# mlelarge/graph_neural_net

Measured on AMD Instinct MI355X. Metric: graph-pairs/sec FGNN fwd+bwd, N=50 regular pairs, higher is better.
Workload: dtype f32

## Files before the change

graph_neural_net_amd/csrc/mlp_fwd.hip:

```cpp
#include "fgnn_common.h"
#include "fgnn_pack.h"

#ifdef FGNN_PHASES
__device__ unsigned long long *g_fwd_stamp = nullptr;
__device__ int g_fwd_sel = 0;
#endif

namespace {

constexpr int TLD = 36;
constexpr int TILE_F = 32 * TLD;

struct TileCtx {
    int g, tt, p, i, jj;
    bool inb;
};

DEVI TileCtx decode_tile(int tile, bool active, int tpg, int N, int P, int j) {
    TileCtx c;
    c.g = __builtin_amdgcn_readfirstlane(active ? tile / tpg : 0);
    c.tt = active ? tile - c.g * tpg : 0;
    c.p = c.tt * FGNN_TILE + j;
    c.inb = active && c.p < P;
    c.i = c.p / N;
    c.jj = c.p - c.i * N;
    return c;
}
DEVI bool tile_valid(const TileCtx &c, int nv) { return c.inb && c.i < nv && c.jj < nv; }

template <int S>
DEVI constexpr int slab_ch(int k, int h) { return S == 16 ? ch_of(k, h) : 2 * k + h; }
template <int S>
DEVI constexpr int slab_kbase(int k) { return S == 16 ? (k & 3) + 8 * (k >> 2) : 2 * k; }
template <int S>
DEVI constexpr int slab_hmul() { return S == 16 ? 4 : 1; }

template <int HMUL>
DEVI int lane_off(const View &v, const TileCtx &c, int h) {
    return c.inb ? HMUL * h * v.ld4 + 4 * c.p : OOB_OFF;
}

template <int S>
DEVI void load_raw(float (&x)[S > 0 ? S : 1], const View &v, const TileCtx &c, int h) {
    if constexpr (S > 0) {
        const int voff = lane_off<slab_hmul<S>()>(v, c, h);
        const int s0 = c.g * v.gs4;
#pragma unroll
        for (int k = 0; k < S; ++k) x[k] = buf_load(v, voff, s0 + slab_kbase<S>(k) * v.ld4);
    }
}

template <int S, bool PK>
DEVI void load_slab(float (&x)[S > 0 ? S : 1], const View &v, const PackedSrc &ps, const TileCtx &c, int h) {
    if constexpr (PK && S == 1) load_packed(x, ps, c, h);
    else load_raw<S>(x, v, c, h);
}

template <int S>
DEVI void apply_norm(float (&x)[S > 0 ? S : 1], const float *rec, bool on, bool valid, int h) {
    if constexpr (S > 0) {
        if (on) {
            const float4 *r4 = reinterpret_cast<const float4 *>(rec);
            const float vf = valid ? 1.f : 0.f;
#pragma unroll
            for (int k = 0; k < S; ++k) {
                const float4 n = r4[slab_ch<S>(k, h)];
                x[k] = ((x[k] - n.x) * n.y + n.z) * vf;
            }
        }
    }
}

template <int CA, int CB>
constexpr int fwd_waves() { return 16; }

template <int CA, int CB, int NMLP, int DEPTH>
struct FwdLayout {
    static constexpr int NW = fwd_waves<CA, CB>();
    static constexpr int SA = CA / 2, SB = CB / 2;
    static constexpr int pad4(int x) { return (x + 3) & ~3; }
    static constexpr PkFwd PK = pk_fwd(CA, CB, DEPTH);
    static constexpr int OFF_W1A = PK.off_w1a;
    static constexpr int OFF_W1B = PK.off_w1b;
    static constexpr int OFF_WH = PK.off_wh;
    static constexpr int BIAS_F = PK.bias_f;
    static constexpr int MLP_STEPS = PK.steps;
    static constexpr int MLP_F = PK.floats;
    static constexpr int WEIGHT_F = NMLP * MLP_F;
    static constexpr int REC_F = 2 * 32 * 4;
    static constexpr int LDS_F = WEIGHT_F + NW * (TILE_F + REC_F);
};

template <int CNT>
DEVI void load_ops(float (&dst)[CNT > 0 ? CNT : 1], const float *wl, int off_steps, int lane) {
    const float4 *p = reinterpret_cast<const float4 *>(wl) + (off_steps / 4) * 64 + lane;
#pragma unroll
    for (int q = 0; q < (CNT + 3) / 4; ++q) {
        const float4 v = p[q * 64];
        if (4 * q + 0 < CNT) dst[4 * q + 0] = v.x;
        if (4 * q + 1 < CNT) dst[4 * q + 1] = v.y;
        if (4 * q + 2 < CNT) dst[4 * q + 2] = v.z;
        if (4 * q + 3 < CNT) dst[4 * q + 3] = v.w;
    }
}

DEVI void load_bias(float (&dst)[16], const float *tail, int layer, int h) {
    const float4 *p = reinterpret_cast<const float4 *>(tail + layer * 32 + h * 16);
#pragma unroll
    for (int q = 0; q < 4; ++q) {
        const float4 v = p[q];
        dst[4 * q + 0] = v.x;
        dst[4 * q + 1] = v.y;
        dst[4 * q + 2] = v.z;
        dst[4 * q + 3] = v.w;
    }
}

template <int CA, int CB, int NMLP, int DEPTH, bool PK, bool SKIP, bool DBG>
DEVI void mlp_fwd_body(const fgnn_mlp_fwd_args A, const int tpg, const int total_tiles, unsigned *const dbg0, unsigned *const dbg1) {
    extern __shared__ __attribute__((aligned(16))) float smem[];
    using L = FwdLayout<CA, CB, NMLP, DEPTH>;
    constexpr int NW = L::NW;
#ifdef FGNN_PHASES
    const unsigned long long st0_ = __builtin_amdgcn_s_memtime();
    unsigned long long st1_ = 0;
    int ntl_ = 0;
#endif
    constexpr int SA = CA / 2, SB = CB / 2;
    const int lane = threadIdx.x & 63, wv = __builtin_amdgcn_readfirstlane(threadIdx.x >> 6);
    const int j = lane & 31, h = lane >> 5;
    const int P = A.N * A.N;
    float *wl = smem;
    float *tl = smem + L::WEIGHT_F + wv * TILE_F;
    float *recA = smem + L::WEIGHT_F + NW * TILE_F + wv * L::REC_F, *recB = recA + 128;
    const View va = make_view(A.a.ptr, A.a.gstride, A.a.ldp, A.G);
    const View vb = make_view(A.b.ptr, A.b.gstride, A.b.ldp, A.G);
    PackedSrc ps = {};
    if constexpr (PK) ps = make_packed_src(A.xbits, A.xdeg, A.G, A.N);
    View vz[NMLP];
#pragma unroll
    for (int m = 0; m < NMLP; ++m) vz[m] = make_view(A.z[m], FGNN_H * A.ldz, A.ldz, A.G);

    const int nwg = gridDim.x;
    const int q = total_tiles / nwg, rem = total_tiles % nwg;
    int T0 = blockIdx.x * q + ((int)blockIdx.x < rem ? (int)blockIdx.x : rem);
    int T1 = T0 + q + ((int)blockIdx.x < rem ? 1 : 0);
    if constexpr (SKIP) {
        T0 = A.ranges[blockIdx.x];
        T1 = A.ranges[blockIdx.x + 1];
    }

    const bool normA = A.a.nrm != nullptr, normB = (CB > 0) && A.b.nrm != nullptr;
    int *live_list = reinterpret_cast<int *>(smem + L::LDS_F);
    int nlive = 0, li = wv, live_cnt = 0;
    bool use_list = false;
    if constexpr (SKIP) {
        nlive = build_live_list(live_list, live_list + LIVE_LIST_CAP, T0, T1, tpg, FGNN_TILE, A.N, A.nvalid, threadIdx.x, 64 * NW);
        use_list = nlive <= LIVE_LIST_CAP;
    }
    auto next_tile = [&](int cur, bool first) {
        if constexpr (SKIP) {
            if (use_list) {
                if (!first) li += NW;
                return __builtin_amdgcn_readfirstlane(li < nlive ? live_list[li] : T1);
            }
            return __builtin_amdgcn_readfirstlane(next_owned_live_tile_p(first ? T0 : cur + 1, T1, live_cnt, wv, NW, tpg, FGNN_TILE, A.N, A.nvalid));
        } else {
            return first ? T0 + wv : cur + NW;
        }
    };
    PkRegs<L::WEIGHT_F / 4, 64 * NW> img;
    if (A.packed) pk_load_regs(img, A.packed);
    __builtin_amdgcn_sched_barrier(0);
    int tile = next_tile(0, true);
    float xa[SA > 0 ? SA : 1], xb[SB > 0 ? SB : 1];
    float4 ra = make_float4(0.f, 0.f, 0.f, 0.f), rb = ra;
    int cached_g = -1, cur_nv = A.N;
    {
        const TileCtx c = decode_tile(tile, tile < T1, tpg, A.N, P, j);
        load_slab<SA, PK>(xa, va, ps, c, h);
        load_slab<SB, PK>(xb, vb, ps, c, h);
        if (tile < T1 && lane < 32) {
            if (normA && lane < CA) {
                ra = reinterpret_cast<const float4 *>(A.a.nrm)[(long long)c.g * A.a.C + lane];
                ra.z = A.a.beta ? A.a.beta[lane] : 0.f;
            }
            if (normB && lane < CB) {
                rb = reinterpret_cast<const float4 *>(A.b.nrm)[(long long)c.g * A.b.C + lane];
                rb.z = A.b.beta ? A.b.beta[lane] : 0.f;
            }
        }
        if (tile < T1) {
            cached_g = c.g;
            cur_nv = __builtin_amdgcn_readfirstlane(nvalid_of(A.nvalid, c.g, A.N));
        }
    }
    if (A.packed) {
        pk_store_regs(wl, img);
    } else {
        constexpr PkFwd pk = L::PK;
#pragma unroll
        for (int m = 0; m < NMLP; ++m) {
            const float *Wp[FGNN_MAX_DEPTH] = {A.W[m][0], A.W[m][1], A.W[m][2]};
            const float *Bp[FGNN_MAX_DEPTH] = {A.bias[m][0], A.bias[m][1], A.bias[m][2]};
            for (int e = threadIdx.x; e < L::MLP_F; e += 64 * NW) {
                if (e < L::BIAS_F) {
                    const int t = e >> 6, l = e & 63;
                    wl[m * L::MLP_F + (t >> 2) * 256 + l * 4 + (t & 3)] = pk_fwd_value(pk, CA, CB, Wp, t, l);
                } else {
                    wl[m * L::MLP_F + e] = pk_bias_value(Bp, e - L::BIAS_F);
                }
            }
        }
    }
    if (lane < 32) {
        reinterpret_cast<float4 *>(recA)[lane] = ra;
        reinterpret_cast<float4 *>(recB)[lane] = rb;
    }
    __syncthreads();
#ifdef FGNN_PHASES
    st1_ = __builtin_amdgcn_s_memtime();
#endif

    while (tile < T1) {
#ifdef FGNN_PHASES
        ++ntl_;
#endif
        const TileCtx c = decode_tile(tile, true, tpg, A.N, P, j);
        if (c.g != cached_g) {
            if (lane < 32) {
                if (normA && lane < CA) {
                    float4 n = reinterpret_cast<const float4 *>(A.a.nrm)[(long long)c.g * A.a.C + lane];
                    n.z = A.a.beta ? A.a.beta[lane] : 0.f;
                    reinterpret_cast<float4 *>(recA)[lane] = n;
                }
                if (normB && lane < CB) {
                    float4 n = reinterpret_cast<const float4 *>(A.b.nrm)[(long long)c.g * A.b.C + lane];
                    n.z = A.b.beta ? A.b.beta[lane] : 0.f;
                    reinterpret_cast<float4 *>(recB)[lane] = n;
                }
            }
            cached_g = c.g;
            cur_nv = __builtin_amdgcn_readfirstlane(nvalid_of(A.nvalid, c.g, A.N));
        }
        const bool c_valid = tile_valid(c, cur_nv);
        const int next = next_tile(tile, false);
        float na[SA > 0 ? SA : 1], nb[SB > 0 ? SB : 1];
        {
            const TileCtx cn = decode_tile(next, next < T1, tpg, A.N, P, j);
            load_slab<SA, PK>(na, va, ps, cn, h);
            load_slab<SB, PK>(nb, vb, ps, cn, h);
        }
        apply_norm<SA>(xa, recA, normA, c_valid, h);
        apply_norm<SB>(xb, recB, normB, c_valid, h);

        const unsigned vmask = (unsigned)__ballot(c_valid);
        const float cnt = (float)__popc(vmask);
        const float inv = cnt > 0.f ? 1.f / cnt : 0.f;
#pragma unroll
        for (int m = 0; m < NMLP; ++m) {
            const float *wm = wl + m * L::MLP_F;
            f32x16 acc;
            {
                float b0[16];
                load_bias(b0, wm + L::BIAS_F, 0, h);
#pragma unroll
                for (int r = 0; r < 16; ++r) acc[r] = b0[r];
                float w1a[SA > 0 ? SA : 1];
                load_ops<SA>(w1a, wm, L::OFF_W1A, lane);
#pragma unroll
                for (int s = 0; s < SA; ++s) acc = mfma32(w1a[s], xa[s], acc);
                if constexpr (SB > 0) {
                    float w1b[SB > 0 ? SB : 1];
                    load_ops<SB>(w1b, wm, L::OFF_W1B, lane);
#pragma unroll
                    for (int s = 0; s < SB; ++s) acc = mfma32(w1b[s], xb[s], acc);
                }
            }
#pragma unroll
            for (int l = 1; l < DEPTH; ++l) {
                float hid[16], bl[16], wh[16];
                load_bias(bl, wm + L::BIAS_F, l, h);
                load_ops<16>(wh, wm, L::OFF_WH + 16 * (l - 1), lane);
                if constexpr (DBG) {
#pragma unroll
                    for (int r = 0; r < 16; ++r) {
                        const unsigned long long mk = __ballot(__float_as_int(acc[r]) > 0);
                        if (lane == 0) {
                            unsigned *o = (m == 0 ? dbg0 : dbg1) + (((long long)c.g * (DEPTH - 1) + (l - 1)) * 32 + ch_of(r, 0)) * tpg + c.tt;
                            o[0] = (unsigned)mk;
                            o[4ll * tpg] = (unsigned)(mk >> 32);
                        }
                    }
                }
#pragma unroll
                for (int r = 0; r < 16; ++r) {
                    hid[r] = relu1(acc[r]);
                    acc[r] = bl[r];
                }
#pragma unroll
                for (int r = 0; r < 16; ++r) acc = mfma32(wh[r], hid[r], acc);
            }
            const int zoff = lane_off<4>(vz[m], c, h);
            const int zs0 = c.g * vz[m].gs4;
#pragma unroll
            for (int r = 0; r < 16; ++r) {
                const int chl = (r & 3) + 8 * (r >> 2);
                const float v = c_valid ? acc[r] : 0.f;
                buf_store(v, vz[m], zoff, zs0 + chl * vz[m].ld4);
                tl[(chl + 4 * h) * TLD + j] = v;
            }
            const float4 *rp = reinterpret_cast<const float4 *>(tl + j * TLD + 16 * h);
            float4 qv[4];
#pragma unroll
            for (int k = 0; k < 4; ++k) qv[k] = rp[k];
            float s = 0.f;
#pragma unroll
            for (int k = 0; k < 4; ++k) s += (qv[k].x + qv[k].y) + (qv[k].z + qv[k].w);
            s += __shfl_xor(s, 32);
            const float mean = s * inv;
            const unsigned mh = vmask >> (16 * h);
            float m2 = 0.f;
#pragma unroll
            for (int k = 0; k < 4; ++k) {
                const float d0 = ((mh >> (4 * k + 0)) & 1u) ? qv[k].x - mean : 0.f;
                const float d1 = ((mh >> (4 * k + 1)) & 1u) ? qv[k].y - mean : 0.f;
                const float d2 = ((mh >> (4 * k + 2)) & 1u) ? qv[k].z - mean : 0.f;
                const float d3 = ((mh >> (4 * k + 3)) & 1u) ? qv[k].w - mean : 0.f;
                m2 += (d0 * d0 + d1 * d1) + (d2 * d2 + d3 * d3);
            }
            m2 += __shfl_xor(m2, 32);
            if (h == 0) {
                float2 o;
                o.x = mean;
                o.y = m2;
                reinterpret_cast<float2 *>(A.part[m])[((long long)c.g * tpg + c.tt) * FGNN_H + j] = o;
            }
        }
        if (lane == 0) A.cnt[(long long)c.g * tpg + c.tt] = cnt;

#pragma unroll
        for (int s = 0; s < SA; ++s) xa[s] = na[s];
#pragma unroll
        for (int s = 0; s < SB; ++s) xb[s] = nb[s];
        tile = next;
    }
    if constexpr (SKIP) {
        for (int t = T0 + wv; t < T1; t += NW) {
            const TileCtx c = decode_tile(t, true, tpg, A.N, P, j);
            if (tile_live(c.tt, A.N, A.nvalid[c.g])) continue;
#pragma unroll
            for (int m = 0; m < NMLP; ++m) {
                if (h == 0)
                    reinterpret_cast<float2 *>(A.part[m])[((long long)c.g * tpg + c.tt) * FGNN_H + j] = make_float2(0.f, 0.f);
            }
            if (lane == 0) A.cnt[(long long)c.g * tpg + c.tt] = 0.f;
        }
    }
#ifdef FGNN_PHASES
    if (g_fwd_stamp && g_fwd_sel == CA * 1000 + CB * 10 + NMLP && (threadIdx.x & 63) == 0) {
        unsigned long long *o = g_fwd_stamp + ((long long)blockIdx.x * NW + wv) * 4;
        o[0] = st0_;
        o[1] = st1_;
        o[2] = __builtin_amdgcn_s_memtime();
        o[3] = ntl_;
    }
#endif
}

template <int CA, int CB, int NMLP, int DEPTH, bool PK = false, bool SKIP = false>
__global__ __launch_bounds__((64 * fwd_waves<CA, CB>()), (fwd_waves<CA, CB>() / 4)) void mlp_fwd_kernel(
    const fgnn_mlp_fwd_args A, const int tpg, const int total_tiles) {
    mlp_fwd_body<CA, CB, NMLP, DEPTH, PK, SKIP, false>(A, tpg, total_tiles, nullptr, nullptr);
}
template <int CA, int CB, int NMLP, int DEPTH, bool PK = false, bool SKIP = false>
__global__ __launch_bounds__((64 * fwd_waves<CA, CB>()), (fwd_waves<CA, CB>() / 4)) void mlp_fwd_dbg_kernel(
    const fgnn_mlp_fwd_args A, const int tpg, const int total_tiles, unsigned *d0, unsigned *d1) {
    mlp_fwd_body<CA, CB, NMLP, DEPTH, PK, SKIP, true>(A, tpg, total_tiles, d0, d1);
}

struct DbgOut {
    unsigned *m[2];
};

template <int CA, int CB, int NMLP, int DEPTH, bool PK = false, bool SKIP = false, bool DBG = false>
int launch_fwd_impl(const fgnn_mlp_fwd_args *a, int tpg, int total, hipStream_t st, const DbgOut &d) {
    using L = FwdLayout<CA, CB, NMLP, DEPTH>;
    constexpr int NW = L::NW;
    constexpr int LDS = (L::LDS_F + (SKIP ? LIVE_LIST_CAP + NW : 0)) * 4;
    static_assert(LDS <= 160 * 1024, "LDS budget");
    static LdsAttrCache attr_cache;
    int grid = (total + NW - 1) / NW;
    const int cap = a->cu_share == 2 ? 128 : 256;
    if (grid > cap) grid = cap;
    if (SKIP) grid = FGNN_RANGE_WG;
    if constexpr (DBG) {
        (void)fgnn_raise_lds(attr_cache, (const void *)mlp_fwd_dbg_kernel<CA, CB, NMLP, DEPTH, PK, SKIP>, LDS);
        hipLaunchKernelGGL((mlp_fwd_dbg_kernel<CA, CB, NMLP, DEPTH, PK, SKIP>), dim3(grid), dim3(64 * NW), LDS, st, *a, tpg, total, d.m[0],
                           d.m[1]);
    } else {
        (void)fgnn_raise_lds(attr_cache, (const void *)mlp_fwd_kernel<CA, CB, NMLP, DEPTH, PK, SKIP>, LDS);
        hipLaunchKernelGGL((mlp_fwd_kernel<CA, CB, NMLP, DEPTH, PK, SKIP>), dim3(grid), dim3(64 * NW), LDS, st, *a, tpg, total);
    }
    FGNN_LAUNCH_CHECK();
    return 0;
}
template <int CA, int CB, int NMLP, int DEPTH, bool PK = false, bool DBG = false>
int launch_fwd(const fgnn_mlp_fwd_args *a, int tpg, int total, hipStream_t st, const DbgOut &d) {
    if (a->ranges) return launch_fwd_impl<CA, CB, NMLP, DEPTH, PK, true, DBG>(a, tpg, total, st, d);
    return launch_fwd_impl<CA, CB, NMLP, DEPTH, PK, false, DBG>(a, tpg, total, st, d);
}

template <int NMLP, int DEPTH, bool DBG = false>
int dispatch_c(const fgnn_mlp_fwd_args *a, int tpg, int total, hipStream_t st, const DbgOut &d = DbgOut{}) {
    const int ca = a->a.C, cb = a->b.C;
    if (a->xbits) {
        if constexpr (DEPTH == 3) {
            if (ca == 2 && cb == 0) return launch_fwd<2, 0, NMLP, DEPTH, true, DBG>(a, tpg, total, st, d);
            if constexpr (NMLP == 1) {
                if (ca == 32 && cb == 2) return launch_fwd<32, 2, NMLP, DEPTH, true, DBG>(a, tpg, total, st, d);
            }
        }
        fgnn_set_error("fgnn_mlp_fwd: xbits needs depth 3 and a 2-channel slab (2 or 32+2 input channels), got depth %d, %d + %d",
                       DEPTH, ca, cb);
        return 1;
    }
#define FGNN_CASE(A_, B_) \
    if (ca == A_ && cb == B_) return launch_fwd<A_, B_, NMLP, DEPTH, false, DBG>(a, tpg, total, st, d);
    FGNN_CASE(2, 0)
    if constexpr (!DBG) {
        FGNN_CASE(16, 0)
    }
    FGNN_CASE(32, 0)
    if constexpr (NMLP == 1) {
        FGNN_CASE(32, 2)
        FGNN_CASE(32, 32)
    }
#undef FGNN_CASE
    fgnn_set_error("fgnn_mlp_fwd: unsupported input channels (%d + %d) for nmlp=%d; built for 2, 16, 32 and, with nmlp=1, 32+2, 32+32", ca, cb, NMLP);
    return 1;
}

}

#ifdef FGNN_PHASES
extern "C" int fgnn_debug_fwd_stamps(void *p, int ca, int cb, int nmlp) {
    const int sel = ca * 1000 + cb * 10 + nmlp;
    if (hipMemcpyToSymbol(HIP_SYMBOL(g_fwd_sel), &sel, sizeof(sel)) != hipSuccess) return 1;
    return hipMemcpyToSymbol(HIP_SYMBOL(g_fwd_stamp), &p, sizeof(p)) == hipSuccess ? 0 : 1;
}
#endif

extern "C" int fgnn_tiles_per_graph(int N) { return (N * N + FGNN_TILE - 1) / FGNN_TILE; }

static int mlp_fwd_entry(const fgnn_mlp_fwd_args *a, void *stream, unsigned *const *dbg) {
    FGNN_CHECK(a != nullptr, "fgnn_mlp_fwd: null args");
    FGNN_CHECK(a->G > 0 && a->N > 0, "fgnn_mlp_fwd: bad G=%d N=%d", a->G, a->N);
    FGNN_CHECK(a->nmlp == 1 || a->nmlp == 2, "fgnn_mlp_fwd: nmlp must be 1 or 2 (got %d)", a->nmlp);
    FGNN_CHECK(a->depth >= 1 && a->depth <= FGNN_MAX_DEPTH, "fgnn_mlp_fwd: depth %d not in 1..%d", a->depth, FGNN_MAX_DEPTH);
    const bool pk_a = a->xbits && a->a.C == 2, pk_b = a->xbits && a->b.C == 2;
    FGNN_CHECK((a->a.ptr || pk_a) && a->a.C > 0, "fgnn_mlp_fwd: slab a missing");
    FGNN_CHECK(a->b.C == 0 || a->b.ptr || pk_b, "fgnn_mlp_fwd: slab b has channels but no pointer");
    FGNN_CHECK(!a->xbits || a->xdeg, "fgnn_mlp_fwd: xbits without xdeg (fgnn_adjacency_degree)");
    FGNN_CHECK((long long)a->N * a->N <= a->ldz && (pk_a || (long long)a->N * a->N <= a->a.ldp), "fgnn_mlp_fwd: channel stride < N*N");
    for (int m = 0; m < a->nmlp; ++m) {
        FGNN_CHECK(a->z[m] && a->part[m], "fgnn_mlp_fwd: missing output %d", m);
        for (int l = 0; l < a->depth; ++l) FGNN_CHECK(a->W[m][l] && a->bias[m][l], "fgnn_mlp_fwd: missing weights mlp %d layer %d", m, l);
    }
    FGNN_CHECK(a->cnt, "fgnn_mlp_fwd: missing cnt");
    FGNN_CHECK(!a->ranges || a->nvalid, "fgnn_mlp_fwd: ranges (fgnn_ragged_tile_ranges) only make sense with nvalid");
    {
        const long long lim = 0x7fffffffll / 4, G = a->G;
        FGNN_CHECK(G * a->a.gstride < lim && G * a->b.gstride < lim && G * FGNN_H * a->ldz < lim,
                   "fgnn_mlp_fwd: a tensor exceeds 2 GiB (32-bit buffer addressing); split the batch");
    }
    const int tpg = fgnn_tiles_per_graph(a->N);
    const long long total = (long long)a->G * tpg;
    FGNN_CHECK(total < (1ll << 30), "fgnn_mlp_fwd: too many tiles");
    hipStream_t st = (hipStream_t)stream;
    if (dbg) {
        FGNN_CHECK(a->depth == 1 || (dbg[0] && (a->nmlp == 1 || dbg[1])), "fgnn_debug_mlp_fwd_masks: one mask buffer per MLP");
        const DbgOut d = {{dbg[0], a->nmlp == 2 ? dbg[1] : nullptr}};
#define FGNN_ND(NM_, D_) \
    if (a->nmlp == NM_ && a->depth == D_) return dispatch_c<NM_, D_, true>(a, tpg, (int)total, st, d);
        FGNN_ND(1, 1) FGNN_ND(1, 2) FGNN_ND(1, 3) FGNN_ND(2, 1) FGNN_ND(2, 2) FGNN_ND(2, 3)
#undef FGNN_ND
    }
#define FGNN_ND(NM_, D_) \
    if (a->nmlp == NM_ && a->depth == D_) return dispatch_c<NM_, D_>(a, tpg, (int)total, st);
    FGNN_ND(1, 1) FGNN_ND(1, 2) FGNN_ND(1, 3) FGNN_ND(2, 1) FGNN_ND(2, 2) FGNN_ND(2, 3)
#undef FGNN_ND
    fgnn_set_error("fgnn_mlp_fwd: unsupported nmlp/depth");
    return 1;
}

extern "C" int fgnn_mlp_fwd(const fgnn_mlp_fwd_args *a, void *stream) { return mlp_fwd_entry(a, stream, nullptr); }

extern "C" int fgnn_debug_mlp_fwd_masks(const fgnn_mlp_fwd_args *a, unsigned *masks0, unsigned *masks1, void *stream) {
    unsigned *const dbg[2] = {masks0, masks1};
    return mlp_fwd_entry(a, stream, dbg);
}
```

Baseline: 42520.

## Defer packed-slab decode and overlap prologue loads with weight staging

```diff
diff --git a/graph_neural_net_amd/csrc/mlp_fwd.hip b/graph_neural_net_amd/csrc/mlp_fwd.hip
--- a/graph_neural_net_amd/csrc/mlp_fwd.hip
+++ b/graph_neural_net_amd/csrc/mlp_fwd.hip
@@ -51,13 +51,54 @@
 }
 
 template <int S, bool PK>
-DEVI void load_slab(float (&x)[S > 0 ? S : 1], const View &v, const PackedSrc &ps, const TileCtx &c, int h) {
-    if constexpr (PK && S == 1) load_packed(x, ps, c, h);
-    else load_raw<S>(x, v, c, h);
-}
-
-template <int S>
-DEVI void apply_norm(float (&x)[S > 0 ? S : 1], const float *rec, bool on, bool valid, int h) {
+constexpr int slab_regs() { return (PK && S == 1) ? 2 : (S > 0 ? S : 1); }
+template <int S, bool PK, int R>
+DEVI void load_slab(float (&x)[R], const View &v, const PackedSrc &ps, const TileCtx &c, int h) {
+    static_assert(R == slab_regs<S, PK>(), "slab register count");
+    if constexpr (PK && S == 1) {
+        const int ob = (c.inb && h == 0) ? (c.i * ps.words + (c.jj >> 5)) * 4 : OOB_OFF;
+        const int od = (c.inb && h == 1 && c.i == c.jj) ? c.i * 4 : OOB_OFF;
+        x[0] = __builtin_bit_cast(float, __builtin_amdgcn_raw_buffer_load_b32(ps.bits, ob, c.g * ps.N * ps.words * 4, 0));
+        x[1] = __builtin_bit_cast(float, __builtin_amdgcn_raw_buffer_load_b32(ps.deg, od, c.g * ps.N * 4, 0));
+    } else {
+        load_raw<S>(x, v, c, h);
+    }
+}
+template <int S, bool PK, int R>
+DEVI void decode_slab(float (&x)[R], const TileCtx &c, int h) {
+    static_assert(R == slab_regs<S, PK>(), "slab register count");
+    if constexpr (PK && S == 1) {
+        const unsigned w = __builtin_bit_cast(unsigned, x[0]);
+        x[0] = h == 0 ? (((w >> (c.jj & 31)) & 1u) ? 1.f : 0.f) : x[1];
+    }
+}
+
+template <int S, bool PK>
+constexpr int slab_loads() { return (PK && S == 1) ? 2 : S; }
+
+struct RecSrc {
+    rsrc_t nrm, beta;
+};
+DEVI RecSrc make_rec_src(const float *nrm, const float *beta, int G, int C) {
+    RecSrc r;
+    long long nb = nrm ? (long long)G * C * 16 : 0;
+    if (nb > 0x7fffffffll) nb = 0x7fffffffll;
+    r.nrm = __builtin_amdgcn_make_buffer_rsrc(const_cast<float *>(nrm), 0, (int)nb, 0x00020000);
+    r.beta = __builtin_amdgcn_make_buffer_rsrc(const_cast<float *>(beta), 0, beta ? C * 4 : 0, 0x00020000);
+    return r;
+}
+DEVI float4 load_rec(const RecSrc &rs, int g, int C, int lane, bool on) {
+    const int vo = on ? lane * 16 : OOB_OFF;
+    float4 r;
+    r.x = __builtin_bit_cast(float, __builtin_amdgcn_raw_buffer_load_b32(rs.nrm, vo, g * C * 16, 0));
+    r.y = __builtin_bit_cast(float, __builtin_amdgcn_raw_buffer_load_b32(rs.nrm, vo, g * C * 16 + 4, 0));
+    r.z = __builtin_bit_cast(float, __builtin_amdgcn_raw_buffer_load_b32(rs.beta, on ? lane * 4 : OOB_OFF, 0, 0));
+    r.w = 0.f;
+    return r;
+}
+
+template <int S, int R>
+DEVI void apply_norm(float (&x)[R], const float *rec, bool on, bool valid, int h) {
     if constexpr (S > 0) {
         if (on) {
             const float4 *r4 = reinterpret_cast<const float4 *>(rec);
@@ -123,10 +164,12 @@
     constexpr int NW = L::NW;
 #ifdef FGNN_PHASES
     const unsigned long long st0_ = __builtin_amdgcn_s_memtime();
-    unsigned long long st1_ = 0;
+    unsigned long long st1_ = 0, stb_ = 0, stm_ = 0;
     int ntl_ = 0;
 #endif
     constexpr int SA = CA / 2, SB = CB / 2;
+    constexpr int TILE_LOADS = slab_loads<SA, PK>() + (SB > 0 ? slab_loads<SB, PK>() : 0);
+    static_assert(TILE_LOADS < 64, "vmcnt is a 6-bit counter");
     const int lane = threadIdx.x & 63, wv = __builtin_amdgcn_readfirstlane(threadIdx.x >> 6);
     const int j = lane & 31, h = lane >> 5;
     const int P = A.N * A.N;
@@ -151,6 +194,7 @@
     }
 
     const bool normA = A.a.nrm != nullptr, normB = (CB > 0) && A.b.nrm != nullptr;
+    const RecSrc rsa = make_rec_src(A.a.nrm, A.a.beta, A.G, A.a.C), rsb = make_rec_src(A.b.nrm, A.b.beta, A.G, A.b.C);
     int *live_list = reinterpret_cast<int *>(smem + L::LDS_F);
     int nlive = 0, li = wv, live_cnt = 0;
     bool use_list = false;
@@ -173,29 +217,26 @@
     if (A.packed) pk_load_regs(img, A.packed);
     __builtin_amdgcn_sched_barrier(0);
     int tile = next_tile(0, true);
-    float xa[SA > 0 ? SA : 1], xb[SB > 0 ? SB : 1];
+    constexpr int RA = slab_regs<SA, PK>(), RB = slab_regs<SB, PK>();
+    float xa[RA], xb[RB];
     float4 ra = make_float4(0.f, 0.f, 0.f, 0.f), rb = ra;
     int cached_g = -1, cur_nv = A.N;
     {
         const TileCtx c = decode_tile(tile, tile < T1, tpg, A.N, P, j);
-        load_slab<SA, PK>(xa, va, ps, c, h);
-        load_slab<SB, PK>(xb, vb, ps, c, h);
-        if (tile < T1 && lane < 32) {
-            if (normA && lane < CA) {
-                ra = reinterpret_cast<const float4 *>(A.a.nrm)[(long long)c.g * A.a.C + lane];
-                ra.z = A.a.beta ? A.a.beta[lane] : 0.f;
-            }
-            if (normB && lane < CB) {
-                rb = reinterpret_cast<const float4 *>(A.b.nrm)[(long long)c.g * A.b.C + lane];
-                rb.z = A.b.beta ? A.b.beta[lane] : 0.f;
-            }
-        }
+        const bool own = tile < T1 && lane < 32;
+        ra = load_rec(rsa, c.g, A.a.C, lane, own && lane < CA);
+        if constexpr (CB > 0) rb = load_rec(rsb, c.g, A.b.C, lane, own && lane < CB);
         if (tile < T1) {
             cached_g = c.g;
             cur_nv = __builtin_amdgcn_readfirstlane(nvalid_of(A.nvalid, c.g, A.N));
         }
+        __builtin_amdgcn_sched_barrier(0);
+        load_slab<SA, PK>(xa, va, ps, c, h);
+        load_slab<SB, PK>(xb, vb, ps, c, h);
+        __builtin_amdgcn_sched_barrier(0);
     }
     if (A.packed) {
+        __builtin_amdgcn_s_waitcnt(0x0F70 | (TILE_LOADS & 15) | ((TILE_LOADS >> 4) << 14));
         pk_store_regs(wl, img);
     } else {
         constexpr PkFwd pk = L::PK;
@@ -217,6 +258,9 @@
         reinterpret_cast<float4 *>(recA)[lane] = ra;
         reinterpret_cast<float4 *>(recB)[lane] = rb;
     }
+#ifdef FGNN_PHASES
+    stb_ = __builtin_amdgcn_s_memtime();
+#endif
     __syncthreads();
 #ifdef FGNN_PHASES
     st1_ = __builtin_amdgcn_s_memtime();
@@ -245,12 +289,14 @@
         }
         const bool c_valid = tile_valid(c, cur_nv);
         const int next = next_tile(tile, false);
-        float na[SA > 0 ? SA : 1], nb[SB > 0 ? SB : 1];
+        float na[RA], nb[RB];
         {
             const TileCtx cn = decode_tile(next, next < T1, tpg, A.N, P, j);
             load_slab<SA, PK>(na, va, ps, cn, h);
             load_slab<SB, PK>(nb, vb, ps, cn, h);
         }
+        decode_slab<SA, PK>(xa, c, h);
+        decode_slab<SB, PK>(xb, c, h);
         apply_norm<SA>(xa, recA, normA, c_valid, h);
         apply_norm<SB>(xb, recB, normB, c_valid, h);
 
@@ -277,6 +323,13 @@
                     for (int s = 0; s < SB; ++s) acc = mfma32(w1b[s], xb[s], acc);
                 }
             }
+#ifdef FGNN_PHASES
+            if (m == 0 && ntl_ == 1) {
+                float t_;
+                asm volatile("v_mov_b32 %0, %1" : "=v"(t_) : "v"(acc[0]));
+                stm_ = __builtin_amdgcn_s_memtime();
+            }
+#endif
 #pragma unroll
             for (int l = 1; l < DEPTH; ++l) {
                 float hid[16], bl[16], wh[16];
@@ -340,9 +393,9 @@
         if (lane == 0) A.cnt[(long long)c.g * tpg + c.tt] = cnt;
 
 #pragma unroll
-        for (int s = 0; s < SA; ++s) xa[s] = na[s];
-#pragma unroll
-        for (int s = 0; s < SB; ++s) xb[s] = nb[s];
+        for (int s = 0; s < RA; ++s) xa[s] = na[s];
+#pragma unroll
+        for (int s = 0; s < (SB > 0 ? RB : 0); ++s) xb[s] = nb[s];
         tile = next;
     }
     if constexpr (SKIP) {
@@ -359,11 +412,13 @@
     }
 #ifdef FGNN_PHASES
     if (g_fwd_stamp && g_fwd_sel == CA * 1000 + CB * 10 + NMLP && (threadIdx.x & 63) == 0) {
-        unsigned long long *o = g_fwd_stamp + ((long long)blockIdx.x * NW + wv) * 4;
+        unsigned long long *o = g_fwd_stamp + ((long long)blockIdx.x * NW + wv) * 8;
         o[0] = st0_;
         o[1] = st1_;
         o[2] = __builtin_amdgcn_s_memtime();
         o[3] = ntl_;
+        o[4] = stb_;
+        o[5] = stm_;
     }
 #endif
 }
```

New measurement: 42630, median of 6. Within noise of the previous version (+0.3%).
